# Saguaro-Biosciences/image-processing-suite

Measured on AMD Instinct MI355X. Metric: fields-of-view/sec, 2080x2080x5ch illum+seg+feat pipe, higher is better.
Workload: dtype fp32 planes / fp64 QC+features / fp32 CPnet (split-fp16 MFMA, f16x3); 1 GPU; configs[1]: 384-well plate, 1 FOV/well, 2080x2080x5ch, illum->seg->feat; batch_per_gpu=48, H=2080, W=2080, C=5, cellpose_model=nuclei, cpnet_weights=cpnet_nuclei_synth.pt, tiles_per_fov=9, parallelism=fov-sharded x1, scheduler=static per-rank steps, steps_this_rank=30, batches_in_flight_per_gpu=2

## Files before the change

### image-processing-suite_amd/csrc/capi.hip

```cpp
#include "cpx_internal.h"
#include <stdarg.h>
#include <stdio.h>
#include <new>

static thread_local char g_err[1024] = {0};

void cpx_set_error(const char* fmt, ...) {
  va_list ap;
  va_start(ap, fmt);
  vsnprintf(g_err, sizeof(g_err), fmt, ap);
  va_end(ap);
}

int cpx_hip_fail(hipError_t e, const char* what) {
  cpx_set_error("HIP error %d (%s) in %s", (int)e, hipGetErrorString(e), what);
  (void)hipGetLastError();
  return e == hipErrorOutOfMemory ? CPX_ERR_OOM : CPX_ERR_HIP;
}

void* cpx_ws(cpx_ctx* ctx, int slot, size_t bytes) {
  if (bytes == 0) bytes = 16;
  if (ctx->ws_bytes[slot] >= bytes) return ctx->ws[slot];
  if (ctx->ws[slot]) {
    (void)hipStreamSynchronize(ctx->stream);
    (void)hipFree(ctx->ws[slot]);
    ctx->ws[slot] = nullptr;
    ctx->ws_bytes[slot] = 0;
  }
  size_t want = bytes + bytes / 4;
  void* p = nullptr;
  hipError_t e = hipMalloc(&p, want);
  if (e != hipSuccess) {
    cpx_hip_fail(e, "workspace hipMalloc");
    return nullptr;
  }
  ctx->ws[slot] = p;
  ctx->ws_bytes[slot] = want;
  ++ctx->ws_gen[slot];
  return p;
}

extern "C" {

int cpx_abi_version(void) { return CPX_ABI_VERSION; }

const char* cpx_last_error(void) { return g_err; }

int cpx_init(int device, cpx_ctx** out) {
  CPX_REQUIRE(out != nullptr, CPX_ERR_ARG, "cpx_init: out is NULL");
  g_err[0] = 0;
  int n = 0;
  CPX_CHECK_HIP(hipGetDeviceCount(&n));
  CPX_REQUIRE(device >= 0 && device < n, CPX_ERR_ARG, "cpx_init: device %d of %d", device, n);
  CPX_CHECK_HIP(hipSetDevice(device));
  cpx_ctx* c = new (std::nothrow) cpx_ctx();
  CPX_REQUIRE(c != nullptr, CPX_ERR_OOM, "cpx_init: host allocation failed");
  c->device = device;
  hipError_t e = hipStreamCreateWithFlags(&c->own_stream, hipStreamNonBlocking);
  if (e != hipSuccess) {
    delete c;
    return cpx_hip_fail(e, "hipStreamCreate");
  }
  c->stream = c->own_stream;
  hipDeviceProp_t prop;
  if (hipGetDeviceProperties(&prop, device) == hipSuccess) c->n_cu = prop.multiProcessorCount;
  *out = c;
  return CPX_OK;
}

void cpx_destroy(cpx_ctx* ctx) {
  if (!ctx) return;
  (void)hipSetDevice(ctx->device);
  if (ctx->stream) (void)hipStreamSynchronize(ctx->stream);
  cpx_fov_free(ctx);
  for (int i = 0; i < kWsSlots; ++i)
    if (ctx->ws[i]) (void)hipFree(ctx->ws[i]);
  if (ctx->own_stream) (void)hipStreamDestroy(ctx->own_stream);
  for (int i = 0; i < cpx_ctx::kGlcmEv; ++i)
    for (int k = 0; k < 2; ++k)
      if (ctx->glcm_ev[i][k]) (void)hipEventDestroy(ctx->glcm_ev[i][k]);
  for (int i = 0; i < cpx_ctx::kSegEv; ++i) {
    for (int k = 0; k < 4; ++k)
      if (ctx->seg_ev[i][k]) (void)hipEventDestroy(ctx->seg_ev[i][k]);
    if (ctx->seg_cnt[i]) (void)hipHostFree(ctx->seg_cnt[i]);
  }
  delete ctx;
}

int cpx_debug_glcm_timing(cpx_ctx* ctx, int enable) {
  CPX_REQUIRE(ctx != nullptr, CPX_ERR_ARG, "cpx_debug_glcm_timing: ctx is NULL");
  if (enable && !ctx->glcm_ev[0][0])
    for (int i = 0; i < cpx_ctx::kGlcmEv; ++i)
      for (int k = 0; k < 2; ++k) CPX_CHECK_HIP(hipEventCreate(&ctx->glcm_ev[i][k]));
  ctx->glcm_timing = enable ? 1 : 0;
  ctx->glcm_nev = 0;
  return CPX_OK;
}

int cpx_debug_glcm_ms(cpx_ctx* ctx, double* ms_out, int* launches_out) {
  CPX_REQUIRE(ctx && ms_out, CPX_ERR_ARG, "cpx_debug_glcm_ms: null argument");
  double ms = 0.0;
  for (int i = 0; i < ctx->glcm_nev; ++i) {
    CPX_CHECK_HIP(hipEventSynchronize(ctx->glcm_ev[i][1]));
    float t = 0.0f;
    CPX_CHECK_HIP(hipEventElapsedTime(&t, ctx->glcm_ev[i][0], ctx->glcm_ev[i][1]));
    ms += t;
  }
  *ms_out = ms;
  if (launches_out) *launches_out = ctx->glcm_nev;
  ctx->glcm_nev = 0;
  return CPX_OK;
}

int cpx_debug_seg_timing(cpx_ctx* ctx, int enable) {
  CPX_REQUIRE(ctx != nullptr, CPX_ERR_ARG, "cpx_debug_seg_timing: ctx is NULL");
  if (enable && !ctx->seg_ev[0][0])
    for (int i = 0; i < cpx_ctx::kSegEv; ++i)
      for (int k = 0; k < 4; ++k) CPX_CHECK_HIP(hipEventCreate(&ctx->seg_ev[i][k]));
  ctx->seg_timing = enable ? 1 : 0;
  ctx->seg_nev = 0;
  return CPX_OK;
}

int cpx_debug_seg_stats(cpx_ctx* ctx, double* follow_ms, double* item_steps, double* fe_reg_ms, int* calls) {
  CPX_REQUIRE(ctx && follow_ms && item_steps && fe_reg_ms, CPX_ERR_ARG, "cpx_debug_seg_stats: null argument");
  double fm = 0.0, st = 0.0, fe = 0.0;
  for (int i = 0; i < ctx->seg_nev; ++i) {
    CPX_CHECK_HIP(hipEventSynchronize(ctx->seg_ev[i][3]));
    float t = 0.0f;
    CPX_CHECK_HIP(hipEventElapsedTime(&t, ctx->seg_ev[i][0], ctx->seg_ev[i][1]));
    fm += t;
    CPX_CHECK_HIP(hipEventElapsedTime(&t, ctx->seg_ev[i][2], ctx->seg_ev[i][3]));
    fe += t;
    const int B = ctx->seg_B[i];
    const int* c = ctx->seg_cnt[i];
    for (int r = 0; r < ctx->seg_rounds[i]; ++r)
      for (int b = 0; b < B; ++b) st += (double)c[r * B + b] * ctx->seg_K[i][r];
  }
  *follow_ms = fm;
  *item_steps = st;
  *fe_reg_ms = fe;
  if (calls) *calls = ctx->seg_nev;
  ctx->seg_nev = 0;
  return CPX_OK;
}

int cpx_debug_flow_error_counts(cpx_ctx* ctx, int out[8]) {
  CPX_REQUIRE(ctx && out, CPX_ERR_ARG, "cpx_debug_flow_error_counts: null argument");
  for (int i = 0; i < 8; ++i) out[i] = 0;
  if (ctx->fe_count_off < 0 || !ctx->ws[WS_SEG_OBJ]) return CPX_OK;
  int c[8];
  CPX_CHECK_HIP(hipMemcpyAsync(c, (const unsigned char*)ctx->ws[WS_SEG_OBJ] + ctx->fe_count_off, sizeof(c),
                               hipMemcpyDeviceToHost, ctx->stream));
  CPX_CHECK_HIP(hipStreamSynchronize(ctx->stream));
  for (int i = 0; i < kFeLists; ++i) out[i] = c[i];
  return CPX_OK;
}

int cpx_debug_flow_error_class(int bh, int bw) { return fe_class(bh, bw); }

int cpx_set_stream(cpx_ctx* ctx, void* hip_stream) {
  CPX_REQUIRE(ctx != nullptr, CPX_ERR_ARG, "cpx_set_stream: ctx is NULL");
  ctx->stream = (hipStream_t)hip_stream;
  if (ctx->own_stream && ctx->stream != ctx->own_stream) {
    (void)hipStreamSynchronize(ctx->own_stream);
    (void)hipStreamDestroy(ctx->own_stream);
    ctx->own_stream = nullptr;
  }
  return CPX_OK;
}

int cpx_sync(cpx_ctx* ctx) {
  CPX_REQUIRE(ctx != nullptr, CPX_ERR_ARG, "cpx_sync: ctx is NULL");
  CPX_CHECK_HIP(hipStreamSynchronize(ctx->stream));
  return CPX_OK;
}

int cpx_stream_create_cu_mask(int device, const uint32_t* cu_mask, int n_words, void** out) {
  CPX_REQUIRE(cu_mask && out && n_words > 0, CPX_ERR_ARG, "cpx_stream_create_cu_mask: bad argument");
  int n = 0;
  CPX_CHECK_HIP(hipGetDeviceCount(&n));
  CPX_REQUIRE(device >= 0 && device < n, CPX_ERR_ARG, "cpx_stream_create_cu_mask: device %d of %d", device, n);
  int prev = 0;
  CPX_CHECK_HIP(hipGetDevice(&prev));
  CPX_CHECK_HIP(hipSetDevice(device));
  hipStream_t s = nullptr;
  const hipError_t e = hipExtStreamCreateWithCUMask(&s, (uint32_t)n_words, cu_mask);
  (void)hipSetDevice(prev);
  if (e != hipSuccess) return cpx_hip_fail(e, "hipExtStreamCreateWithCUMask");
  *out = (void*)s;
  return CPX_OK;
}

int cpx_stream_destroy(void* stream) {
  CPX_REQUIRE(stream != nullptr, CPX_ERR_ARG, "cpx_stream_destroy: stream is NULL");
  CPX_CHECK_HIP(hipStreamSynchronize((hipStream_t)stream));
  CPX_CHECK_HIP(hipStreamDestroy((hipStream_t)stream));
  return CPX_OK;
}

}

extern "C" int cpx_reserve(cpx_ctx* ctx, int max_planes, int H, int W, int max_fovs,
                           int max_label) {
  CPX_REQUIRE(ctx != nullptr, CPX_ERR_ARG, "cpx_reserve: ctx is NULL");
  CPX_REQUIRE(max_planes > 0 && H > 0 && W > 0 && max_fovs >= 0 && max_label >= 0, CPX_ERR_ARG,
              "cpx_reserve: bad sizes");
  if (!cpx_ws(ctx, WS_PARTIALS, (size_t)48 * 64 * max_planes)) return CPX_ERR_OOM;
  const int K = std::max(std::min(H, W) / 8, 1);
  const int nr = std::max(K - 2, 1);
  if (!cpx_ws(ctx, WS_QC_ROWS, (size_t)16 * max_planes * H * K)) return CPX_ERR_OOM;
  size_t ring = (size_t)8 * max_planes * K * nr;
  ring = ((ring + 255) / 256) * 256 + (size_t)8 * max_planes + 256;
  if (!cpx_ws(ctx, WS_QC_RINGS, ring)) return CPX_ERR_OOM;
  if (!cpx_ws(ctx, WS_QC_MISC, (size_t)16 * (H + W) + 256)) return CPX_ERR_OOM;
  return CPX_OK;
}
```

### image-processing-suite_amd/csrc/k_seg.hip

```cpp
#include "cpx_internal.h"
#include <stdlib.h>
#include <limits.h>
#include <math.h>
#include <stdio.h>
#include <type_traits>
#include <vector>

#pragma clang fp contract(off)

namespace {

constexpr int kT = 256;
constexpr int kRpad = 20;

__device__ __forceinline__ unsigned int f2key(float f) {
  unsigned int u = __float_as_uint(f);
  return (u & 0x80000000u) ? ~u : (u | 0x80000000u);
}
__device__ __forceinline__ float key2f(unsigned int k) {
  unsigned int u = (k & 0x80000000u) ? (k & 0x7fffffffu) : ~k;
  return __uint_as_float(u);
}
__device__ __forceinline__ unsigned short f2bf16(float f) {
  unsigned int u = __float_as_uint(f);
// ... 198 lines not shown
      static_cast<float*>(tiles)[(ntile * npx + q) * nchan + ch] = out;
    else
      static_cast<unsigned short*>(tiles)[(ntile * npx + q) * nchan + ch] = f2bf16(out);
  }
}

__global__ __launch_bounds__(kT) void k_seg_average(const void* __restrict__ net, int layout, int nout,
                                                    cpx_seg_geom g, const float* __restrict__ taper,
                                                    float* __restrict__ yf) {
  const int fov = blockIdx.y;
  const int q = blockIdx.x * kT + threadIdx.x;
  if (q >= g.Ly * g.Lx) return;
  const int y = q / g.Lx, x = q - y * g.Lx;
  const int py = y + g.py0, px = x + g.px0;
  const int npx = g.by * g.bx;
  float acc[4] = {0.f, 0.f, 0.f, 0.f};
  float nav = 0.0f;
  for (int jy = 0; jy < g.ny; ++jy) {
    const int ty = py - g.ys[jy];
    if (ty < 0 || ty >= g.by) continue;
    for (int jx = 0; jx < g.nx; ++jx) {
      const int tx = px - g.xs[jx];
      if (tx < 0 || tx >= g.bx) continue;
      const long long t = (long long)fov * g.ny * g.nx + jy * g.nx + jx;
      const int o = ty * g.bx + tx;
      const float m = taper[o];
      for (int c = 0; c < nout && c < 4; ++c) {
        float v;
        if (layout == CPX_TILE_F32_NCHW) v = static_cast<const float*>(net)[(t * nout + c) * npx + o];
        else if (layout == CPX_TILE_F32_NHWC) v = static_cast<const float*>(net)[(t * npx + o) * nout + c];
        else v = bf162f(static_cast<const unsigned short*>(net)[(t * npx + o) * nout + c]);
        acc[c] = acc[c] + v * m;
      }
      nav = nav + m;
    }
  }
  for (int c = 0; c < nout && c < 4; ++c)
    yf[(((long long)fov * nout + c) * g.Ly + y) * g.Lx + x] = acc[c] / nav;
}

struct DynBufs {
  float2* dps;
  float2* dpf;
  float2* p;
  unsigned char* mov;
  int* h;
  unsigned int* M;
  unsigned char* sflag;
  int* m0;
  int ms;
  int* seeds;
  int* cnt;
  int* first;
  int* newlab;
  unsigned char* mark;
  int* marklist;
  int* act;
  void* fitems0;
  void* fitems1;
  int* fcnt;
  int* tiles;
  int* totals;
  cpx_seg_stats* st;
};

constexpr int kPrepPer = 8;

template <bool RESAMPLE>
__global__ __launch_bounds__(kT) void k_dyn_prep(const float* __restrict__ yf, int Ly, int Lx,
                                                 int Dy, int Dx, AxisTab uy, AxisTab ux,
                                                 DynBufs d) {
  const int fov = blockIdx.y;
  const long long n = (long long)Dy * Dx;
  const long long nl = (long long)Ly * Lx;
  const long long q0 = (long long)blockIdx.x * kT * kPrepPer;
  const float* f = yf + (long long)fov * 3 * nl;
  unsigned int movbits = 0;
#pragma unroll
  for (int k = 0; k < kPrepPer; ++k) {
    const long long q = q0 + k * kT + threadIdx.x;
    if (q >= n) break;
    float v[3];
    if (RESAMPLE) {
      const int qi = (int)q;
      const int y = qi / Dx, x = qi - y * Dx;
      const int y0 = uy.i0[y], y1 = uy.i1[y], x0 = ux.i0[x], x1 = ux.i1[x];
      const float wy = uy.w[y], wx = ux.w[x];
#pragma unroll
      for (int c = 0; c < 3; ++c) {
        const float* P = f + c * nl;
        const float r0 = P[y0 * Lx + x0] * (1.0f - wx) + P[y0 * Lx + x1] * wx;
        const float r1 = P[y1 * Lx + x0] * (1.0f - wx) + P[y1 * Lx + x1] * wx;
        v[c] = r0 * (1.0f - wy) + r1 * wy;
      }
    } else {
#pragma unroll
      for (int c = 0; c < 3; ++c) v[c] = f[c * nl + q];
    }
    const float cp = v[2] > 0.0f ? 1.0f : 0.0f;
    const float dy = (v[0] * cp) / 5.0f, dx = (v[1] * cp) / 5.0f;
    d.dps[(long long)fov * n + q] = make_float2(dy, dx);
    d.dpf[(long long)fov * n + q] = make_float2(v[0], v[1]);
    const bool moving = fabsf(dy) > 1e-3f;
    d.mov[(long long)fov * n + q] = (unsigned char)moving;
    movbits |= (unsigned int)moving << k;
  }
  __shared__ int wsum[kPrepPer][kT / 64];
  __shared__ int sbase;
  const int lane = threadIdx.x & 63, wid = threadIdx.x >> 6;
  unsigned long long bal[kPrepPer];
#pragma unroll
  for (int k = 0; k < kPrepPer; ++k) {
    bal[k] = __ballot((movbits >> k) & 1u);
    if (lane == 0) wsum[k][wid] = __popcll(bal[k]);
  }
  __syncthreads();
  if (threadIdx.x == 0) {
    int s = 0;
    for (int k = 0; k < kPrepPer; ++k)
      for (int w = 0; w < kT / 64; ++w) {
        const int c = wsum[k][w];
        wsum[k][w] = s;
        s += c;
      }
    sbase = s ? atomicAdd(&d.st[fov].n_moving, s) : 0;
  }
  __syncthreads();
  const unsigned long long lower = (1ull << lane) - 1ull;
#pragma unroll
  for (int k = 0; k < kPrepPer; ++k)
    if ((movbits >> k) & 1u)
      d.act[(long long)fov * n + sbase + wsum[k][wid] + __popcll(bal[k] & lower)] =
          (int)(q0 + k * kT + threadIdx.x);
}

__device__ __forceinline__ void agg_add(int* base, int key, bool valid) {
  const int lane = threadIdx.x & 63;
  unsigned long long pend = __ballot(valid);
  while (pend) {
    const int leader = __ffsll((long long)pend) - 1;
    const int k0 = __shfl(key, leader);
    const unsigned long long m = __ballot(valid && key == k0);
    if (lane == leader) atomicAdd(&base[k0], __popcll(m));
    pend &= ~m;
  }
}

struct FollowItem {
  int q;
  float py, px;
  int pad;
};

template <int NI, bool V4>
__global__ __launch_bounds__(kT) void k_dyn_follow(int Dy, int Dx, int niter, int step0, int K,
                                                   int from_act, const FollowItem* __restrict__ in,
                                                   const int* __restrict__ in_cnt,
                                                   FollowItem* __restrict__ out,
                                                   int* __restrict__ out_cnt, DynBufs d) {
  const int fov = blockIdx.y;
  const long long n = (long long)Dy * Dx;
  const int n_moving = d.st[fov].n_moving;
  if (n_moving < 5) return;
  const int n_in = from_act ? n_moving : in_cnt[fov];
  const int steps = min(K, niter - step0);
  const float2* __restrict__ I = d.dps + (long long)fov * n;
  float2* __restrict__ P = d.p + (long long)fov * n;
  const FollowItem* src = in + (long long)fov * n;
  FollowItem* dst = out + (long long)fov * n;
  const float fLy = (float)(Dy - 1), fLx = (float)(Dx - 1);
  const int lane = threadIdx.x & 63, wid = threadIdx.x >> 6;
  const int Dxh = Dx + 2 * kRpad;
  int* Hh = d.h + (long long)fov * (Dy + 2 * kRpad) * Dxh;
  const unsigned char* Ib = reinterpret_cast<const unsigned char*>(I);
  const __amdgpu_buffer_rsrc_t rsI =
      __builtin_amdgcn_make_buffer_rsrc(const_cast<float2*>(I), (short)0, (int)(8 * n), 0x00020000);
  (void)rsI;
  __shared__ int wsum[NI][kT / 64];
  __shared__ int sbase;
  for (int i0 = blockIdx.x * kT * NI; i0 < n_in; i0 += gridDim.x * kT * NI) {
    bool active[NI], done[NI];
    int q[NI];
    float py[NI], px[NI];
#pragma unroll
    for (int j = 0; j < NI; ++j) {
      const int i = i0 + j * kT + threadIdx.x;
      active[j] = i < n_in;
      q[j] = 0;
      py[j] = 0.0f;
      px[j] = 0.0f;
      if (active[j]) {
        if (from_act) {
          q[j] = d.act[(long long)fov * n + i];
          py[j] = (float)(q[j] / Dx);
          px[j] = (float)(q[j] % Dx);
        } else {
          const FollowItem it = src[i];
          q[j] = it.q;
          py[j] = it.py;
          px[j] = it.px;
        }
      }
      done[j] = !active[j];
    }
    float2 af[NI], bf[NI], cf[NI], ef[NI];
    int cy[NI], cx[NI];
#pragma unroll
    for (int j = 0; j < NI; ++j) {
      cy[j] = -1;
      cx[j] = -1;
      af[j] = bf[j] = cf[j] = ef[j] = make_float2(0.0f, 0.0f);
    }
    for (int s = 0; s < steps; ++s) {
      bool all = true;
#pragma unroll
      for (int j = 0; j < NI; ++j) all = all && done[j];
      if (all) break;
      int yi[NI], xi[NI];
#pragma unroll
      for (int j = 0; j < NI; ++j) {
        yi[j] = (int)py[j];
        xi[j] = (int)px[j];
        if (yi[j] == cy[j] && xi[j] == cx[j]) continue;
        cy[j] = yi[j];
        cx[j] = xi[j];
        const int y0 = min(Dy - 1, max(0, yi[j])), x0 = min(Dx - 1, max(0, xi[j]));
        const unsigned int b00 = 8u * (unsigned int)(y0 * Dx + x0);
        const unsigned int bdx = x0 + 1 < Dx ? 8u : 0u, bdy = y0 + 1 < Dy ? 8u * (unsigned int)Dx : 0u;
        if constexpr (V4) {
          const unsigned int o = bdx ? b00 : b00 - 8u;
          const float4 r0 = __builtin_bit_cast(float4, __builtin_amdgcn_raw_buffer_load_b128(rsI, o, 0, 0));
          const float4 r1 = __builtin_bit_cast(float4, __builtin_amdgcn_raw_buffer_load_b128(rsI, o + bdy, 0, 0));
          af[j] = bdx ? make_float2(r0.x, r0.y) : make_float2(r0.z, r0.w);
          bf[j] = make_float2(r0.z, r0.w);
          cf[j] = bdx ? make_float2(r1.x, r1.y) : make_float2(r1.z, r1.w);
          ef[j] = make_float2(r1.z, r1.w);
        } else {
          af[j] = *reinterpret_cast<const float2*>(Ib + b00);
          bf[j] = *reinterpret_cast<const float2*>(Ib + (b00 + bdx));
          cf[j] = *reinterpret_cast<const float2*>(Ib + (b00 + bdy));
          ef[j] = *reinterpret_cast<const float2*>(Ib + (b00 + bdy + bdx));
        }
      }
#pragma unroll
      for (int j = 0; j < NI; ++j) {
        const double2 a = {(double)af[j].x, (double)af[j].y}, b = {(double)bf[j].x, (double)bf[j].y},
                      c = {(double)cf[j].x, (double)cf[j].y}, e = {(double)ef[j].x, (double)ef[j].y};
        double vy, vx;
        if (py[j] >= 1.0f && px[j] >= 1.0f) {
          const float yf = py[j] - (float)yi[j], xf = px[j] - (float)xi[j];
          const double y1 = (double)yf, x1 = (double)xf, y0d = (double)(1.0f - yf), x0d = (double)(1.0f - xf);
          const double w00 = y0d * x0d, w01 = y0d * x1, w10 = y1 * x0d, w11 = y1 * x1;
          vy = a.x * w00 + b.x * w01 + c.x * w10 + e.x * w11;
          vx = a.y * w00 + b.y * w01 + c.y * w10 + e.y * w11;
        } else {
          const double yy = (double)py[j] - (double)yi[j], xx = (double)px[j] - (double)xi[j];
          vy = a.x * (1.0 - yy) * (1.0 - xx) + b.x * (1.0 - yy) * xx + c.x * yy * (1.0 - xx) + e.x * yy * xx;
          vx = a.y * (1.0 - yy) * (1.0 - xx) + b.y * (1.0 - yy) * xx + c.y * yy * (1.0 - xx) + e.y * yy * xx;
        }
        const float ny = __builtin_amdgcn_fmed3f(py[j] + (float)vy, 0.0f, fLy);
        const float nx = __builtin_amdgcn_fmed3f(px[j] + (float)vx, 0.0f, fLx);
        if (!done[j]) {
          if (ny == py[j] && nx == px[j]) done[j] = true;
          py[j] = ny;
          px[j] = nx;
        }
      }
    }
    const bool last = step0 + steps >= niter;
    bool carry[NI];
    unsigned long long bal[NI];
#pragma unroll
    for (int j = 0; j < NI; ++j) {
      const bool fin = active[j] && (done[j] || last);
      agg_add(Hh, ((int)py[j] + kRpad) * Dxh + (int)px[j] + kRpad, fin);
    }
#pragma unroll
    for (int j = 0; j < NI; ++j) {
      if (active[j] && (done[j] || last)) P[q[j]] = make_float2(py[j], px[j]);
      carry[j] = active[j] && !done[j] && !last;
      bal[j] = __ballot(carry[j]);
      if (lane == 0) wsum[j][wid] = __popcll(bal[j]);
    }
    __syncthreads();
    if (threadIdx.x == 0) {
      int t = 0;
      for (int j = 0; j < NI; ++j)
        for (int w = 0; w < kT / 64; ++w) {
          const int c = wsum[j][w];
          wsum[j][w] = t;
          t += c;
        }
      sbase = t ? atomicAdd(&out_cnt[fov], t) : 0;
    }
    __syncthreads();
#pragma unroll
    for (int j = 0; j < NI; ++j)
      if (carry[j]) {
        FollowItem it;
        it.q = q[j];
        it.py = py[j];
        it.px = px[j];
        it.pad = 0;
        dst[sbase + wsum[j][wid] + __popcll(bal[j] & ((1ull << lane) - 1ull))] = it;
      }
    __syncthreads();
  }
}

constexpr int kPx4 = 4;

__global__ __launch_bounds__(kT) void k_hist_init(int Dy, int Dx, DynBufs d) {
  const int fov = blockIdx.y;
  const int Dxh = Dx + 2 * kRpad, Dyh = Dy + 2 * kRpad;
  const long long nh = (long long)Dyh * Dxh;
  const long long b0 = ((long long)blockIdx.x * kT + threadIdx.x) * kPx4;
  if (b0 >= nh) return;
  const unsigned char* mov = d.mov + (long long)fov * Dy * Dx;
  int v[kPx4];
#pragma unroll
  for (int u = 0; u < kPx4; ++u) {
    const long long b = b0 + u;
    v[u] = 0;
    if (b < nh) {
      const int bi = (int)b;
      const int y = bi / Dxh - kRpad, x = bi - (bi / Dxh) * Dxh - kRpad;
      if (y >= 0 && y < Dy && x >= 0 && x < Dx) v[u] = mov[(long long)y * Dx + x] ? 0 : 1;
    }
  }
  int* h = d.h + (long long)fov * nh;
  if ((nh & 3) == 0) {
    *reinterpret_cast<int4*>(h + b0) = make_int4(v[0], v[1], v[2], v[3]);
  } else {
#pragma unroll
    for (int u = 0; u < kPx4; ++u)
      if (b0 + u < nh) h[b0 + u] = v[u];
  }
}

__global__ __launch_bounds__(kT) void k_hist_moving(int Dy, int Dx, DynBufs d) {
  const int fov = blockIdx.y;
  const long long n = (long long)Dy * Dx;
  const int i = blockIdx.x * kT + threadIdx.x;
  const int n_moving = d.st[fov].n_moving;
  if (n_moving >= 5 || (long long)blockIdx.x * kT >= n_moving) return;
  const int Dxh = Dx + 2 * kRpad;
  const bool valid = i < n_moving;
  int key = 0;
  if (valid) {
    const int q = d.act[(long long)fov * n + i];
    float2 pp = n_moving >= 5 ? d.p[(long long)fov * n + q] : make_float2((float)(q / Dx), (float)(q % Dx));
    key = ((int)pp.x + kRpad) * Dxh + (int)pp.y + kRpad;
  }
  agg_add(d.h + (long long)fov * (Dy + 2 * kRpad) * Dxh, key, valid);
}

__global__ __launch_bounds__(kT) void k_seed_flags(int Dyh, int Dxh, DynBufs d) {
  const int fov = blockIdx.y;
  const long long nh = (long long)Dyh * Dxh;
  const long long q0 = ((long long)blockIdx.x * kT + threadIdx.x) * kPx4;
  if (q0 >= nh) return;
  const int* h = d.h + (long long)fov * nh;
  const bool vec = (nh & 3) == 0;
  int v[kPx4];
  if (vec) {
    const int4 t = *reinterpret_cast<const int4*>(h + q0);
    v[0] = t.x;
    v[1] = t.y;
    v[2] = t.z;
    v[3] = t.w;
  } else {
#pragma unroll
    for (int u = 0; u < kPx4; ++u) v[u] = q0 + u < nh ? h[q0 + u] : 0;
  }
  unsigned int fw = 0;
#pragma unroll
  for (int u = 0; u < kPx4; ++u) {
    if (v[u] <= 10) continue;
    const long long q = q0 + u;
    const int y = (int)(q / Dxh), x = (int)(q % Dxh);
    int mx = v[u];
    for (int dy = -2; dy <= 2; ++dy)
      for (int dx = -2; dx <= 2; ++dx) {
        int yy = y + dy, xx = x + dx;
        yy = yy < 0 ? -yy - 1 : (yy >= Dyh ? 2 * Dyh - yy - 1 : yy);
        xx = xx < 0 ? -xx - 1 : (xx >= Dxh ? 2 * Dxh - xx - 1 : xx);
        mx = max(mx, h[(long long)yy * Dxh + xx]);
      }
    fw |= (unsigned int)(v[u] >= mx) << (8 * u);
  }
  unsigned char* f = d.sflag + (long long)fov * nh;
  if (vec && ((((uintptr_t)(f + q0)) & 3u) == 0)) {
    *reinterpret_cast<unsigned int*>(f + q0) = fw;
  } else {
#pragma unroll
    for (int u = 0; u < kPx4; ++u)
      if (q0 + u < nh) f[q0 + u] = (unsigned char)((fw >> (8 * u)) & 1u);
  }
}

constexpr int kOcThreads = 256;
constexpr int kOcPer = 32;
constexpr int kOcTile = kOcThreads * kOcPer;

__device__ __forceinline__ int oc_load(const unsigned char* f, long long n, long long i0,
                                       unsigned int* bits) {
  unsigned int b = 0;
  if (i0 + kOcPer <= n && (((uintptr_t)(f + i0)) & 15u) == 0) {
    const uint4* v = reinterpret_cast<const uint4*>(f + i0);
#pragma unroll
    for (int h = 0; h < 2; ++h) {
      const uint4 t = v[h];
      const unsigned int w[4] = {t.x, t.y, t.z, t.w};
#pragma unroll
      for (int k = 0; k < 4; ++k)
#pragma unroll
        for (int by = 0; by < 4; ++by)
          b |= (((w[k] >> (8 * by)) & 0xffu) ? 1u : 0u) << (h * 16 + k * 4 + by);
    }
  } else {
    for (int j = 0; j < kOcPer; ++j)
      if (i0 + j < n && f[i0 + j]) b |= 1u << j;
  }
  *bits = b;
  return __popc(b);
}

__global__ __launch_bounds__(kOcThreads) void k_oc_count(const unsigned char* __restrict__ flags,
                                                         long long n, int ntile, int* __restrict__ tiles) {
  const int fov = blockIdx.y, t = blockIdx.x;
  const unsigned char* f = flags + (long long)fov * n;
  unsigned int bits;
  int c = oc_load(f, n, (long long)t * kOcTile + (long long)threadIdx.x * kOcPer, &bits);
  c = wave_sum(c);
  __shared__ int ws[kOcThreads / 64];
  if ((threadIdx.x & 63) == 0) ws[threadIdx.x >> 6] = c;
  __syncthreads();
  if (threadIdx.x == 0) {
    int s = 0;
    for (int w = 0; w < kOcThreads / 64; ++w) s += ws[w];
    tiles[(long long)fov * ntile + t] = s;
  }
}

__global__ __launch_bounds__(1024) void k_oc_scan(int ntile, int* __restrict__ tiles,
                                                  int* __restrict__ totals) {
  const int fov = blockIdx.x;
  int* t = tiles + (long long)fov * ntile;
  __shared__ int wsum[16];
  __shared__ int base;
  if (threadIdx.x == 0) base = 0;
  __syncthreads();
  const int lane = threadIdx.x & 63, wid = threadIdx.x >> 6;
  for (int i0 = 0; i0 < ntile; i0 += 1024) {
    const int i = i0 + threadIdx.x;
    const int v = i < ntile ? t[i] : 0;
    int inc = v;
// ... 1453 lines not shown
  if (!buf) return CPX_ERR_OOM;
  int* base = (int*)buf;
  t.ty.i0 = base;
  t.ty.i1 = base + Ly;
  t.ty.w = (const float*)(base + 2 * Ly);
  t.tx.i0 = base + 3 * Ly;
  t.tx.i1 = base + 3 * Ly + Lx;
  t.tx.w = (const float*)(base + 3 * Ly + 2 * Lx);
  t.ynear = base + 3 * Ly + 3 * Lx;
  t.xnear = base + 3 * Ly + 3 * Lx + H;
  int* up = base + 3 * Ly + 3 * Lx + H + W;
  t.uy.i0 = up;
  t.uy.i1 = up + H;
  t.uy.w = (const float*)(up + 2 * H);
  t.ux.i0 = up + 3 * H;
  t.ux.i1 = up + 3 * H + W;
  t.ux.w = (const float*)(up + 3 * H + 2 * W);
  const int key[6] = {H, W, Ly, Lx, 2, 0};
  bool same = ctx->seg_gen == ctx->ws_gen[WS_SEG_TAB];
  for (int i = 0; i < 6; ++i) same = same && ctx->seg_key[i] == key[i];
  if (same) return CPX_OK;
  std::vector<int> h(words);
  axis_coeffs(H, Ly, &h[0], &h[Ly], (float*)&h[2 * Ly]);
  axis_coeffs(W, Lx, &h[3 * Ly], &h[3 * Ly + Lx], (float*)&h[3 * Ly + 2 * Lx]);
  const double ify = 1.0 / ((double)H / (double)Ly), ifx = 1.0 / ((double)W / (double)Lx);
  for (int y = 0; y < H; ++y) h[3 * Ly + 3 * Lx + y] = std::min((int)floor(y * ify), Ly - 1);
  for (int x = 0; x < W; ++x) h[3 * Ly + 3 * Lx + H + x] = std::min((int)floor(x * ifx), Lx - 1);
  const size_t u = (size_t)3 * Ly + 3 * Lx + H + W;
  axis_coeffs(Ly, H, &h[u], &h[u + H], (float*)&h[u + 2 * H]);
  axis_coeffs(Lx, W, &h[u + 3 * H], &h[u + 3 * H + W], (float*)&h[u + 3 * H + 2 * W]);
  CPX_CHECK_HIP(hipMemcpyAsync(buf, h.data(), words * 4, hipMemcpyHostToDevice, ctx->stream));
  CPX_CHECK_HIP(hipStreamSynchronize(ctx->stream));
  for (int i = 0; i < 6; ++i) ctx->seg_key[i] = key[i];
  ctx->seg_gen = ctx->ws_gen[WS_SEG_TAB];
  return CPX_OK;
}

bool geom_ok(const cpx_seg_geom* g) {
  if (!g || g->Ly <= 0 || g->Lx <= 0 || g->by <= 0 || g->bx <= 0) return false;
  if (g->ny < 1 || g->nx < 1 || g->ny > CPX_SEG_MAX_TILES_AXIS || g->nx > CPX_SEG_MAX_TILES_AXIS) return false;
  for (int i = 0; i < g->ny; ++i)
    if (g->ys[i] < 0 || g->ys[i] + g->by > g->Lyp) return false;
  for (int i = 0; i < g->nx; ++i)
    if (g->xs[i] < 0 || g->xs[i] + g->bx > g->Lxp) return false;
  return g->py0 >= 0 && g->px0 >= 0 && g->py0 + g->Ly <= g->Lyp && g->px0 + g->Lx <= g->Lxp;
}

}

extern "C" int cpx_seg_percentiles(cpx_ctx* ctx, const float* corr_dev, int B, int C, int H, int W,
                                   int nchan, double* pct_dev) {
  CPX_REQUIRE(ctx && corr_dev && pct_dev, CPX_ERR_ARG, "cpx_seg_percentiles: null argument");
  CPX_REQUIRE(B > 0 && C > 0 && nchan > 0 && nchan <= C && H > 0 && W > 0 && B * nchan <= 65535,
              CPX_ERR_ARG, "cpx_seg_percentiles: bad sizes");
  const int P = B * nchan;
  const size_t hist_bytes = (size_t)P * 4 * 2048 * 4;
  unsigned char* ws = (unsigned char*)cpx_ws(ctx, WS_SEG_PCT, hist_bytes + sizeof(PctState) * P + 256);
  if (!ws) return CPX_ERR_OOM;
  unsigned int* hist = (unsigned int*)ws;
  PctState* st = (PctState*)(ws + hist_bytes);
  const long long N = (long long)H * W;
  for (int pass = 0; pass < 3; ++pass) {
    CPX_CHECK_HIP(hipMemsetAsync(hist, 0, hist_bytes, ctx->stream));
    hipLaunchKernelGGL(k_pct_hist, dim3(48, P), dim3(kT), 0, ctx->stream, corr_dev, C, N, nchan,
                       pass, (const PctState*)st, hist);
    CPX_CHECK_LAUNCH("k_pct_hist");
    hipLaunchKernelGGL(k_pct_find, dim3(P), dim3(256), 0, ctx->stream, N, pass, st,
                       (const unsigned int*)hist, pct_dev);
    CPX_CHECK_LAUNCH("k_pct_find");
  }
  return CPX_OK;
}

extern "C" int cpx_seg_tiles(cpx_ctx* ctx, const float* corr_dev, int B, int C, int H, int W,
                             int nchan, const double* pct_dev, const cpx_seg_geom* geom, int layout,
                             void* tiles_dev) {
  CPX_REQUIRE(ctx && corr_dev && pct_dev && tiles_dev, CPX_ERR_ARG, "cpx_seg_tiles: null argument");
  CPX_REQUIRE(geom_ok(geom), CPX_ERR_ARG, "cpx_seg_tiles: bad geometry");
  CPX_REQUIRE(B > 0 && B <= 65535 && nchan > 0 && nchan <= C && H > 0 && W > 0, CPX_ERR_ARG,
              "cpx_seg_tiles: bad sizes");
  CPX_REQUIRE(layout == CPX_TILE_F32_NCHW || layout == CPX_TILE_BF16_NHWC || layout == CPX_TILE_F32_NHWC,
              CPX_ERR_ARG, "cpx_seg_tiles: bad layout %d", layout);
  SegTabs t;
  int rc = seg_tables(ctx, H, W, geom->Ly, geom->Lx, t);
  if (rc) return rc;
  const int npx = geom->by * geom->bx;
  hipLaunchKernelGGL(k_seg_tiles, dim3(cpx_div_up(npx, kT), geom->ny * geom->nx, B), dim3(kT), 0,
                     ctx->stream, corr_dev, C, H, W, nchan, pct_dev, *geom, t.ty, t.tx, layout,
                     tiles_dev);
  CPX_CHECK_LAUNCH("k_seg_tiles");
  return CPX_OK;
}

extern "C" int cpx_seg_average(cpx_ctx* ctx, const void* net_dev, int layout, int B, int nout,
                               const cpx_seg_geom* geom, const float* taper_dev, float* yf_dev) {
  CPX_REQUIRE(ctx && net_dev && taper_dev && yf_dev, CPX_ERR_ARG, "cpx_seg_average: null argument");
  CPX_REQUIRE(geom_ok(geom), CPX_ERR_ARG, "cpx_seg_average: bad geometry");
  CPX_REQUIRE(B > 0 && B <= 65535 && nout > 0 && nout <= 4, CPX_ERR_ARG, "cpx_seg_average: bad sizes");
  hipLaunchKernelGGL(k_seg_average, dim3(cpx_div_up(geom->Ly * geom->Lx, kT), B), dim3(kT), 0,
                     ctx->stream, net_dev, layout, nout, *geom, taper_dev, yf_dev);
  CPX_CHECK_LAUNCH("k_seg_average");
  return CPX_OK;
}

static int ordered_compact(cpx_ctx* ctx, const unsigned char* flags, long long n, int B, int* tiles,
                           int* totals, int cap, int* out, long long out_stride) {
  const int ntile = cpx_div_up(n, kOcTile);
  hipLaunchKernelGGL(k_oc_count, dim3(ntile, B), dim3(kOcThreads), 0, ctx->stream, flags, n, ntile, tiles);
  hipLaunchKernelGGL(k_oc_scan, dim3(B), dim3(1024), 0, ctx->stream, ntile, tiles, totals);
  hipLaunchKernelGGL(k_oc_emit, dim3(ntile, B), dim3(kOcThreads), 0, ctx->stream, flags, n, ntile,
                     (const int*)tiles, cap, out, out_stride);
  CPX_CHECK_LAUNCH("ordered_compact");
  return CPX_OK;
}

__global__ void k_seed_count(int B, int ms, const int* __restrict__ totals, cpx_seg_stats* __restrict__ st) {
  const int fov = blockIdx.x * blockDim.x + threadIdx.x;
  if (fov >= B) return;
  const int t = totals[fov];
  st[fov].n_seeds = min(t, ms);
  st[fov].n_seeds_found = t;
  if (t > ms) atomicOr(&st[fov].overflow, CPX_SEG_OVF_SEEDS);
}

extern "C" int cpx_seg_masks(cpx_ctx* ctx, const float* yf_dev, int B, const cpx_seg_geom* geom,
                             int H, int W, int niter, double flow_threshold, int min_size,
                             int max_objects, int resample, int32_t* labels_dev,
                             cpx_seg_stats* stats_dev) {
  CPX_REQUIRE(ctx && yf_dev && labels_dev && stats_dev, CPX_ERR_ARG, "cpx_seg_masks: null argument");
  CPX_REQUIRE(geom_ok(geom), CPX_ERR_ARG, "cpx_seg_masks: bad geometry");
  CPX_REQUIRE(B > 0 && B <= 65535 && H > 0 && W > 0 && niter >= 0 && max_objects > 0 &&
                  (long long)(H + 2 * kRpad) * (W + 2 * kRpad) < (1LL << 31) &&
                  (long long)H * W * (long long)sizeof(float2) < (1LL << 32),
              CPX_ERR_ARG, "cpx_seg_masks: bad sizes");
  const int Ly = geom->Ly, Lx = geom->Lx;
  const int Dy = resample ? H : Ly, Dx = resample ? W : Lx;
  const int Dyh = Dy + 2 * kRpad, Dxh = Dx + 2 * kRpad;
  const long long n = (long long)Dy * Dx, nh = (long long)Dyh * Dxh;
  SegTabs tabs;
  int rc = seg_tables(ctx, H, W, Ly, Lx, tabs);
  if (rc) return rc;
  auto al = [](size_t b) { return (b + 255) / 256 * 256; };
  const int ntile = cpx_div_up(std::max(n, nh), kOcTile);
  const size_t sz_f2 = al(sizeof(float2) * B * n);
  const size_t sz_d2 = al(sizeof(float2) * B * n);
  const size_t sz_b = al((size_t)B * n);
  const size_t sz_h = al(sizeof(int) * B * nh), sz_hb = al((size_t)B * nh);
  const size_t sz_m0 = resample ? 0 : al(sizeof(int) * B * n);
  const int ms = max_objects;
  const size_t sz_seeds = al(sizeof(int) * (size_t)B * ms);
  const size_t sz_cnt = al(sizeof(int) * (size_t)B * (ms + 1));
  const size_t sz_act = al(sizeof(int) * B * n);
  const size_t sz_small = al(sizeof(int) * (size_t)B);
  constexpr int k0 = 16, sw = 384, k1 = 128;
  const int rounds = cpx_div_up(sw, k0) + cpx_div_up(std::max(0, niter - sw), k1) + 2;
  const size_t sz_fcnt = al(sizeof(int) * (size_t)B * (rounds + 1));
  const size_t sz_items = al((size_t)16 * B * n);
  const size_t sz_tiles = al(sizeof(int) * (size_t)B * ntile);
  const size_t total = sz_d2 + 2 * sz_f2 + 2 * sz_b + 2 * sz_h + sz_hb + sz_m0 + 2 * sz_seeds + 3 * sz_cnt +
                       sz_act + sz_small + sz_tiles + sz_fcnt + 2 * sz_items;
  unsigned char* w = (unsigned char*)cpx_ws(ctx, WS_SEG_DYN, total);
  if (!w) return CPX_ERR_OOM;
  DynBufs d;
  d.dps = (float2*)w; w += sz_d2;
  d.dpf = (float2*)w; w += sz_f2;
  d.p = (float2*)w; w += sz_f2;
  d.mov = w; w += sz_b;
  d.mark = w; w += sz_b;
  d.h = (int*)w; w += sz_h;
  d.M = (unsigned int*)w; w += sz_h;
  d.sflag = w; w += sz_hb;
  d.m0 = resample ? labels_dev : (int*)w; w += sz_m0;
  d.seeds = (int*)w; w += sz_seeds;
  d.marklist = (int*)w; w += sz_seeds;
  d.cnt = (int*)w; w += sz_cnt;
  d.first = (int*)w; w += sz_cnt;
  d.newlab = (int*)w; w += sz_cnt;
  d.act = (int*)w; w += sz_act;
  d.fcnt = (int*)w; w += sz_fcnt;
  d.fitems0 = w; w += sz_items;
  d.fitems1 = w; w += sz_items;
  d.totals = (int*)w; w += sz_small;
  d.tiles = (int*)w; w += sz_tiles;
  d.st = stats_dev;
  d.ms = ms;
  CPX_CHECK_HIP(hipMemsetAsync(stats_dev, 0, sizeof(cpx_seg_stats) * B, ctx->stream));
  CPX_CHECK_HIP(hipMemsetAsync(d.M, 0, sz_h, ctx->stream));
  CPX_CHECK_HIP(hipMemsetAsync(d.mark, 0, sz_b, ctx->stream));
  CPX_CHECK_HIP(hipMemsetAsync(d.cnt, 0, sz_cnt, ctx->stream));
  CPX_CHECK_HIP(hipMemsetAsync(d.first, 0x7f, sz_cnt, ctx->stream));
  CPX_CHECK_HIP(hipMemsetAsync(d.newlab, 0, sz_cnt, ctx->stream));
  CPX_CHECK_HIP(hipMemsetAsync(d.fcnt, 0, sz_fcnt, ctx->stream));
  const dim3 gp(cpx_div_up(n, kT), B), gh(cpx_div_up(nh, kT), B);
  const dim3 gprep(cpx_div_up(n, (long long)kT * kPrepPer), B);
  if (resample)
    hipLaunchKernelGGL(k_dyn_prep<true>, gprep, dim3(kT), 0, ctx->stream, yf_dev, Ly, Lx, Dy, Dx,
                       tabs.uy, tabs.ux, d);
  else
    hipLaunchKernelGGL(k_dyn_prep<false>, gprep, dim3(kT), 0, ctx->stream, yf_dev, Ly, Lx, Dy, Dx,
                       tabs.uy, tabs.ux, d);
  const dim3 gh4(cpx_div_up(nh, (long long)kT * kPx4), B), gp4(cpx_div_up(n, (long long)kT * kPx4), B);
  hipLaunchKernelGGL(k_hist_init, gh4, dim3(kT), 0, ctx->stream, Dy, Dx, d);
  const int sev = ctx->seg_timing && ctx->seg_nev < cpx_ctx::kSegEv ? ctx->seg_nev++ : -1;
  bool fe_timed = false;
  if (sev >= 0) CPX_CHECK_HIP(hipEventRecord(ctx->seg_ev[sev][0], ctx->stream));
  {
    const int fblk = std::max(1, std::min(cpx_div_up(n, kT), (16 * ctx->n_cu + B - 1) / B));
    int step = 0, r = 0;
    do {
      const int K = step < sw ? k0 : k1;
      const FollowItem* in = (const FollowItem*)(r & 1 ? d.fitems1 : d.fitems0);
      FollowItem* out = (FollowItem*)(r & 1 ? d.fitems0 : d.fitems1);
      const bool v4 = Dx >= 2 && 8LL * n < (1LL << 31);
      auto kern = v4 ? k_dyn_follow<2, true> : k_dyn_follow<2, false>;
      hipLaunchKernelGGL(kern, dim3(fblk, B), dim3(kT), 0, ctx->stream, Dy, Dx, niter, step, K,
                         r == 0 ? 1 : 0, in, (const int*)(d.fcnt + (size_t)B * r), out,
                         d.fcnt + (size_t)B * (r + 1), d);
      if (sev >= 0 && r < 64) ctx->seg_K[sev][r] = std::min(K, std::max(niter - step, 0));
      step += K;
      ++r;
    } while (step < niter);
    if (sev >= 0) {
      CPX_CHECK_HIP(hipEventRecord(ctx->seg_ev[sev][1], ctx->stream));
      const int rr = std::min(r, 64);
      const int need = B * rr;
      if (ctx->seg_cnt_cap[sev] < need) {
        if (ctx->seg_cnt[sev]) CPX_CHECK_HIP(hipHostFree(ctx->seg_cnt[sev]));
        CPX_CHECK_HIP(hipHostMalloc((void**)&ctx->seg_cnt[sev], sizeof(int) * need));
        ctx->seg_cnt_cap[sev] = need;
      }
      CPX_CHECK_HIP(hipMemcpy2DAsync(ctx->seg_cnt[sev], sizeof(int), stats_dev, sizeof(cpx_seg_stats),
                                     sizeof(int), B, hipMemcpyDeviceToHost, ctx->stream));
      if (rr > 1)
        CPX_CHECK_HIP(hipMemcpyAsync(ctx->seg_cnt[sev] + B, d.fcnt + B, sizeof(int) * B * (rr - 1),
                                     hipMemcpyDeviceToHost, ctx->stream));
      ctx->seg_B[sev] = B;
      ctx->seg_rounds[sev] = rr;
    }
  }
  hipLaunchKernelGGL(k_hist_moving, dim3(1, B), dim3(kT), 0, ctx->stream, Dy, Dx, d);
  hipLaunchKernelGGL(k_seed_flags, gh4, dim3(kT), 0, ctx->stream, Dyh, Dxh, d);
  CPX_CHECK_LAUNCH("cpx_seg_masks follow");
  rc = ordered_compact(ctx, d.sflag, nh, B, d.tiles, d.totals, ms, d.seeds, ms);
  if (rc) return rc;
  hipLaunchKernelGGL(k_seed_count, dim3(cpx_div_up(B, 256)), dim3(256), 0, ctx->stream, B, ms,
                     (const int*)d.totals, stats_dev);
  hipLaunchKernelGGL(k_seed_expand, dim3(std::max(1, (4 * ctx->n_cu + B - 1) / B), B), dim3(kT), 0,
                     ctx->stream, Dyh, Dxh, d);
  hipLaunchKernelGGL(k_assign, dim3(cpx_div_up(n, (long long)kT * kAsg), B), dim3(kT), 0, ctx->stream, Dy, Dx, d);
  hipLaunchKernelGGL(k_relabel_mark, dim3(cpx_div_up(ms, kT), B), dim3(kT), 0, ctx->stream, Dy, Dx, d);
  CPX_CHECK_LAUNCH("cpx_seg_masks seeds");
  rc = ordered_compact(ctx, d.mark, n, B, d.tiles, d.totals, ms, d.marklist, ms);
  if (rc) return rc;
  hipLaunchKernelGGL(k_relabel_apply, dim3(4, B), dim3(kT), 0, ctx->stream, Dy, Dx, d);
  hipLaunchKernelGGL(k_apply_newlab, gp4, dim3(kT), 0, ctx->stream, Dy, Dx, d);
  CPX_CHECK_LAUNCH("cpx_seg_masks relabel");
  const int ML = max_objects;
  const size_t sz_lst = al(sizeof(cpx_label_stats) * (size_t)B * (ML + 1));
  const size_t sz_obj = al(sizeof(cpx_object) * (size_t)B * ML);
  const size_t sz_hdr = al(sizeof(cpx_fov_objects) * (size_t)B);
  const size_t sz_bad = al((size_t)B * (ML + 1));
  const size_t sz_l2i = al(sizeof(int) * (size_t)B * (ML + 1));
  const size_t sz_abs = al(sizeof(int) * (size_t)B * ML);
  const size_t sz_nl = sz_abs;
  constexpr int kFeQueues = 6;
  const size_t sz_fec = al(sizeof(int) * (8 + kFeQueues));
  const size_t sz_fel = al(sizeof(int2) * (size_t)kFeLists * B * ML);
  const size_t gscr_per = (size_t)2 * (Dy + 2) * (Dx + 2);
  const size_t sz_gscr = al(sizeof(double) * B * gscr_per);
  unsigned char* o = (unsigned char*)cpx_ws(ctx, WS_SEG_OBJ,
      sz_lst + sz_obj + sz_hdr + sz_bad + sz_l2i + sz_abs + sz_nl + sz_fec + sz_fel + sz_gscr);
  if (!o) return CPX_ERR_OOM;
  cpx_label_stats* lst = (cpx_label_stats*)o; o += sz_lst;
  cpx_object* obj = (cpx_object*)o; o += sz_obj;
  cpx_fov_objects* hdr = (cpx_fov_objects*)o; o += sz_hdr;
  unsigned char* bad = o; o += sz_bad;
  int* l2i = (int*)o; o += sz_l2i;
  int* absorber = (int*)o; o += sz_abs;
  int* newlab = (int*)o; o += sz_nl;
  int* fec = (int*)o; o += sz_fec;
  int2* fel = (int2*)o; o += sz_fel;
  double* gscr = (double*)o;
  ctx->fe_count_off = -1;
  if (flow_threshold > 0.0) {
    rc = cpx_objects(ctx, d.m0, B, Dy, Dx, ML, 0, lst, obj, hdr);
    if (rc) return rc;
    CPX_CHECK_HIP(hipMemsetAsync(bad, 0, sz_bad, ctx->stream));
    CPX_CHECK_HIP(hipMemsetAsync(fec, 0, sizeof(int) * (8 + kFeQueues), ctx->stream));
    const cpx_fe_lists lists = {fec, fel, (long long)B * ML};
    int* const fq = fec + 8;
    ctx->fe_count_off = (unsigned char*)fec - (unsigned char*)ctx->ws[WS_SEG_OBJ];
    hipLaunchKernelGGL(k_fe_classify, dim3(cpx_div_up(ML, 256), B), dim3(256), 0, ctx->stream, ML,
                       (const cpx_object*)obj, (const cpx_fov_objects*)hdr, lists);
    if (sev >= 0) CPX_CHECK_HIP(hipEventRecord(ctx->seg_ev[sev][2], ctx->stream));
    rc = cpx_flow_error_reg_launch(ctx->n_cu, ctx->stream, d.m0, (const float2*)d.dpf, Dy, Dx, ML, obj, lists,
                                   fq, flow_threshold, bad);
    if (rc) return rc;
    if (sev >= 0) {
      CPX_CHECK_HIP(hipEventRecord(ctx->seg_ev[sev][3], ctx->stream));
      fe_timed = true;
    }
    hipLaunchKernelGGL((k_flow_error_lds<kFeLargeThreads / 2, kFeLargeCells, 2 * kFeU, float, 4>),
                       dim3(2 * ctx->n_cu), dim3(kFeLargeThreads / 2), 0, ctx->stream, (const int*)d.m0,
                       (const float2*)d.dpf, Dy, Dx, ML, (const cpx_object*)obj, lists, fq + 3, flow_threshold,
                       bad);
    hipLaunchKernelGGL(k_flow_error_tail, dim3(ctx->n_cu), dim3(kFeLargeThreads), 0, ctx->stream,
                       (const int*)d.m0, (const float2*)d.dpf, Dy, Dx, ML, (const cpx_object*)obj, lists,
                       fq + 4, flow_threshold, bad);
    {
      const int nbig = std::max(1, std::min(ctx->n_cu, 4 * B));
      const long long slice = (long long)(B * gscr_per / nbig) & ~1LL;
      hipLaunchKernelGGL(k_flow_error_big, dim3(nbig), dim3(kBigThreads), 0, ctx->stream,
                         (const int*)d.m0, (const float2*)d.dpf, Dy, Dx, ML, (const cpx_object*)obj, lists,
                         fq + 5, flow_threshold, gscr, slice, bad);
    }
    hipLaunchKernelGGL(k_flow_error_fov, dim3(B), dim3(kFlowThreads), 0, ctx->stream,
                       (const int*)d.m0, (const float2*)d.dpf, Dy, Dx, ML, (const cpx_object*)obj, lists,
                       flow_threshold, gscr, (long long)gscr_per, bad);
    hipLaunchKernelGGL(k_apply_bad, gp4, dim3(kT), 0, ctx->stream, n, ML,
                       (const unsigned char*)bad, d.m0);
    hipLaunchKernelGGL(k_count_bad, dim3(B), dim3(256), 0, ctx->stream, ML,
                       (const unsigned char*)bad, (const int*)fq, kFeQueues, stats_dev);
    CPX_CHECK_LAUNCH("cpx_seg_masks flow error");
  }
  if (!resample) {
    hipLaunchKernelGGL(k_upsample, dim3(cpx_div_up(W, kT), cpx_div_up(H, kUpRows), B), dim3(kT), 0,
                       ctx->stream, (const int*)d.m0, Ly, Lx, H, W, tabs.ynear, tabs.xnear, labels_dev);
    CPX_CHECK_LAUNCH("k_upsample");
  }
  rc = cpx_objects(ctx, labels_dev, B, H, W, ML, 0, lst, obj, hdr);
  if (rc) return rc;
  const long long N = (long long)H * W;
  const size_t sz_fill = al(sizeof(int) * (size_t)B * N);
  const size_t sz_fscr = al(sizeof(unsigned int) * 2 * (size_t)B * ((W + 31) / 32) * H);
  unsigned char* fw = (unsigned char*)cpx_ws(ctx, WS_SEG_FILL, sz_fill + sz_fscr);
  if (!fw) return CPX_ERR_OOM;
  int* fillidx = (int*)fw;
  unsigned int* fscr = (unsigned int*)(fw + sz_fill);
  CPX_CHECK_HIP(hipMemsetAsync(fillidx, 0, sizeof(int) * (size_t)B * N, ctx->stream));
  CPX_CHECK_HIP(hipMemsetAsync(absorber, 0x7f, sz_abs, ctx->stream));
  CPX_CHECK_HIP(hipMemsetAsync(l2i, 0, sz_l2i, ctx->stream));
  hipLaunchKernelGGL(k_lab2idx, dim3(cpx_div_up(ML, kT), B), dim3(kT), 0, ctx->stream, ML,
                     (const cpx_object*)obj, (const cpx_fov_objects*)hdr, l2i);
  static bool fattr = false;
  const size_t flds = sizeof(unsigned int) * 2 * kFillMaxWords;
  if (!fattr) {
    CPX_CHECK_HIP(hipFuncSetAttribute((const void*)k_fill_holes,
                                      hipFuncAttributeMaxDynamicSharedMemorySize, (int)flds));
    CPX_CHECK_HIP(hipFuncSetAttribute((const void*)k_fill_seq,
                                      hipFuncAttributeMaxDynamicSharedMemorySize, (int)flds));
    fattr = true;
  }
  hipLaunchKernelGGL(k_fill_holes, dim3(std::max(1, std::min(ML, (2 * ctx->n_cu + B - 1) / B)), B),
                     dim3(kFillThreads), flds, ctx->stream,
                     (const int*)labels_dev, H, W, ML, min_size, (const cpx_object*)obj,
                     (const cpx_fov_objects*)hdr, (const int*)l2i, fillidx, absorber);
  hipLaunchKernelGGL(k_fill_holes_big, dim3(B), dim3(1024), 0, ctx->stream,
                     (const int*)labels_dev, H, W, ML, min_size, (const cpx_object*)obj,
                     (const cpx_fov_objects*)hdr, (const int*)l2i, fillidx, absorber, fscr);
  if (sev >= 0 && !fe_timed) {
    CPX_CHECK_HIP(hipEventRecord(ctx->seg_ev[sev][2], ctx->stream));
    CPX_CHECK_HIP(hipEventRecord(ctx->seg_ev[sev][3], ctx->stream));
  }
  hipLaunchKernelGGL(k_fill_final, dim3(B), dim3(1024), 0, ctx->stream, ML, min_size,
                     (const cpx_object*)obj, (const cpx_fov_objects*)hdr, (const int*)absorber,
                     (const int*)labels_dev, (const int*)fillidx, W, N, newlab, stats_dev);
  hipLaunchKernelGGL(k_fill_apply, dim3(std::max(1, std::min(cpx_div_up(N, kT), 8 * ctx->n_cu / B + 1)), B),
// ... 9 lines not shown
```

Baseline: 501.6 FOV/s.

## Restructure Cellpose flow-follow loop with wave ballots, packed loads and occupancy bound

Reworks the per-step flow-following kernel. Per-thread done flags become wave-level ballot masks so the loop exits once no lane in the wave is moving. Bilinear samples are kept in two float4 registers and reloaded only when the cell index changes, with the V4 path dropping clamping in favour of __umul24 address math and a wave-uniform right-edge fixup. The kernel gets a launch-bounds minimum-waves hint and uses mbcnt for compaction offsets. This aims to cut VALU work, redundant loads and register pressure in the hot iteration, but relies on positions staying in range, since the clamp is removed, and the occupancy hint may cause spills.

```diff
diff --git a/image-processing-suite_amd/csrc/capi.hip b/image-processing-suite_amd/csrc/capi.hip
--- a/image-processing-suite_amd/csrc/capi.hip
+++ b/image-processing-suite_amd/csrc/capi.hip
@@ -117,6 +117,7 @@
   if (enable && !ctx->seg_ev[0][0])
     for (int i = 0; i < cpx_ctx::kSegEv; ++i)
       for (int k = 0; k < 4; ++k) CPX_CHECK_HIP(hipEventCreate(&ctx->seg_ev[i][k]));
+  for (int i = 0; i < ctx->seg_nev; ++i) CPX_CHECK_HIP(hipEventSynchronize(ctx->seg_ev[i][3]));
   ctx->seg_timing = enable ? 1 : 0;
   ctx->seg_nev = 0;
   return CPX_OK;
diff --git a/image-processing-suite_amd/csrc/k_seg.hip b/image-processing-suite_amd/csrc/k_seg.hip
--- a/image-processing-suite_amd/csrc/k_seg.hip
+++ b/image-processing-suite_amd/csrc/k_seg.hip
@@ -374,13 +374,24 @@
   int pad;
 };
 
+typedef float FollowQuad __attribute__((ext_vector_type(4)));
+
+#ifndef CPX_FOLLOW_NI
+#define CPX_FOLLOW_NI 2
+#endif
+#ifndef CPX_FOLLOW_K0
+#define CPX_FOLLOW_K0 16
+#endif
+#ifndef CPX_FOLLOW_WAVES
+#define CPX_FOLLOW_WAVES 8
+#endif
+
 template <int NI, bool V4>
-__global__ __launch_bounds__(kT) void k_dyn_follow(int Dy, int Dx, int niter, int step0, int K,
-                                                   int from_act, const FollowItem* __restrict__ in,
-                                                   const int* __restrict__ in_cnt,
-                                                   FollowItem* __restrict__ out,
-                                                   int* __restrict__ out_cnt, DynBufs d) {
+__global__ __launch_bounds__(kT, V4 ? CPX_FOLLOW_WAVES : 1) void k_dyn_follow(
+    int Dy, int Dx, int niter, int step0, int K, int from_act, const FollowItem* __restrict__ in,
+    const int* __restrict__ in_cnt, FollowItem* __restrict__ out, int* __restrict__ out_cnt, DynBufs d) {
   const int fov = blockIdx.y;
+  const int bx = blockIdx.x, nbx = gridDim.x;
   const long long n = (long long)Dy * Dx;
   const int n_moving = d.st[fov].n_moving;
   if (n_moving < 5) return;
@@ -391,6 +402,8 @@
   const FollowItem* src = in + (long long)fov * n;
   FollowItem* dst = out + (long long)fov * n;
   const float fLy = (float)(Dy - 1), fLx = (float)(Dx - 1);
+  const int Dym1 = Dy - 1, Dxm1 = Dx - 1;
+  const unsigned int Dx8 = 8u * (unsigned int)Dx;
   const int lane = threadIdx.x & 63, wid = threadIdx.x >> 6;
   const int Dxh = Dx + 2 * kRpad;
   int* Hh = d.h + (long long)fov * (Dy + 2 * kRpad) * Dxh;
@@ -400,10 +413,11 @@
   (void)rsI;
   __shared__ int wsum[NI][kT / 64];
   __shared__ int sbase;
-  for (int i0 = blockIdx.x * kT * NI; i0 < n_in; i0 += gridDim.x * kT * NI) {
-    bool active[NI], done[NI];
+  for (int i0 = bx * kT * NI; i0 < n_in; i0 += nbx * kT * NI) {
+    bool active[NI];
     int q[NI];
     float py[NI], px[NI];
+    unsigned long long moving[NI], act[NI];
 #pragma unroll
     for (int j = 0; j < NI; ++j) {
       const int i = i0 + j * kT + threadIdx.x;
@@ -423,54 +437,78 @@
           px[j] = it.px;
         }
       }
-      done[j] = !active[j];
-    }
-    float2 af[NI], bf[NI], cf[NI], ef[NI];
-    int cy[NI], cx[NI];
+      act[j] = moving[j] = __ballot(active[j]);
+    }
+    FollowQuad r0[NI], r1[NI];
+    unsigned int cb[NI];
 #pragma unroll
     for (int j = 0; j < NI; ++j) {
-      cy[j] = -1;
-      cx[j] = -1;
-      af[j] = bf[j] = cf[j] = ef[j] = make_float2(0.0f, 0.0f);
+      cb[j] = 0xffffffffu;
+      r0[j] = r1[j] = FollowQuad{0.0f, 0.0f, 0.0f, 0.0f};
     }
     for (int s = 0; s < steps; ++s) {
-      bool all = true;
-#pragma unroll
-      for (int j = 0; j < NI; ++j) all = all && done[j];
-      if (all) break;
+      unsigned long long any = 0;
+#pragma unroll
+      for (int j = 0; j < NI; ++j) any |= moving[j];
+      if (any == 0) break;
       int yi[NI], xi[NI];
+      unsigned int o0[NI], o1[NI];
+      bool changed[NI], redge[NI];
 #pragma unroll
       for (int j = 0; j < NI; ++j) {
         yi[j] = (int)py[j];
         xi[j] = (int)px[j];
-        if (yi[j] == cy[j] && xi[j] == cx[j]) continue;
-        cy[j] = yi[j];
-        cx[j] = xi[j];
-        const int y0 = min(Dy - 1, max(0, yi[j])), x0 = min(Dx - 1, max(0, xi[j]));
-        const unsigned int b00 = 8u * (unsigned int)(y0 * Dx + x0);
-        const unsigned int bdx = x0 + 1 < Dx ? 8u : 0u, bdy = y0 + 1 < Dy ? 8u * (unsigned int)Dx : 0u;
+        unsigned int b00;
+        int y0 = yi[j], x0 = xi[j];
         if constexpr (V4) {
-          const unsigned int o = bdx ? b00 : b00 - 8u;
-          const float4 r0 = __builtin_bit_cast(float4, __builtin_amdgcn_raw_buffer_load_b128(rsI, o, 0, 0));
-          const float4 r1 = __builtin_bit_cast(float4, __builtin_amdgcn_raw_buffer_load_b128(rsI, o + bdy, 0, 0));
-          af[j] = bdx ? make_float2(r0.x, r0.y) : make_float2(r0.z, r0.w);
-          bf[j] = make_float2(r0.z, r0.w);
-          cf[j] = bdx ? make_float2(r1.x, r1.y) : make_float2(r1.z, r1.w);
-          ef[j] = make_float2(r1.z, r1.w);
+          b00 = 8u * (__umul24((unsigned int)y0, (unsigned int)Dx) + (unsigned int)x0);
         } else {
-          af[j] = *reinterpret_cast<const float2*>(Ib + b00);
-          bf[j] = *reinterpret_cast<const float2*>(Ib + (b00 + bdx));
-          cf[j] = *reinterpret_cast<const float2*>(Ib + (b00 + bdy));
-          ef[j] = *reinterpret_cast<const float2*>(Ib + (b00 + bdy + bdx));
+          y0 = min(Dy - 1, max(0, y0));
+          x0 = min(Dx - 1, max(0, x0));
+          b00 = 8u * (unsigned int)(y0 * Dx + x0);
         }
+        changed[j] = b00 != cb[j];
+        cb[j] = b00;
+        redge[j] = x0 >= Dxm1;
+        o0[j] = (V4 && redge[j]) ? b00 - 8u : b00;
+        o1[j] = y0 < Dym1 ? o0[j] + Dx8 : o0[j];
       }
 #pragma unroll
       for (int j = 0; j < NI; ++j) {
-        const double2 a = {(double)af[j].x, (double)af[j].y}, b = {(double)bf[j].x, (double)bf[j].y},
-                      c = {(double)cf[j].x, (double)cf[j].y}, e = {(double)ef[j].x, (double)ef[j].y};
+        if (!changed[j]) continue;
+        if constexpr (V4) {
+          r0[j] = __builtin_bit_cast(FollowQuad, __builtin_amdgcn_raw_buffer_load_b128(rsI, o0[j], 0, 0));
+          r1[j] = __builtin_bit_cast(FollowQuad, __builtin_amdgcn_raw_buffer_load_b128(rsI, o1[j], 0, 0));
+        } else {
+          const unsigned int bdx = redge[j] ? 0u : 8u;
+          const float2 a = *reinterpret_cast<const float2*>(Ib + o0[j]);
+          const float2 b = *reinterpret_cast<const float2*>(Ib + (o0[j] + bdx));
+          const float2 c = *reinterpret_cast<const float2*>(Ib + o1[j]);
+          const float2 e = *reinterpret_cast<const float2*>(Ib + (o1[j] + bdx));
+          r0[j] = FollowQuad{a.x, a.y, b.x, b.y};
+          r1[j] = FollowQuad{c.x, c.y, e.x, e.y};
+        }
+      }
+#pragma unroll
+      for (int j = 0; j < NI; ++j) asm volatile("" : "+v"(r0[j]), "+v"(r1[j]));
+#pragma unroll
+      for (int j = 0; j < NI; ++j) {
+        if constexpr (V4) {
+          if (__builtin_amdgcn_ballot_w64(px[j] >= fLx) != 0) {
+            asm volatile("" : "+v"(r0[j]), "+v"(r1[j]));
+            if (px[j] >= fLx) {
+              r0[j].x = r0[j].z;
+              r0[j].y = r0[j].w;
+              r1[j].x = r1[j].z;
+              r1[j].y = r1[j].w;
+            }
+          }
+        }
+        const double2 a = {(double)r0[j].x, (double)r0[j].y}, b = {(double)r0[j].z, (double)r0[j].w},
+                      c = {(double)r1[j].x, (double)r1[j].y}, e = {(double)r1[j].z, (double)r1[j].w};
         double vy, vx;
         if (py[j] >= 1.0f && px[j] >= 1.0f) {
-          const float yf = py[j] - (float)yi[j], xf = px[j] - (float)xi[j];
+          const float yf = __builtin_amdgcn_fractf(py[j]), xf = __builtin_amdgcn_fractf(px[j]);
           const double y1 = (double)yf, x1 = (double)xf, y0d = (double)(1.0f - yf), x0d = (double)(1.0f - xf);
           const double w00 = y0d * x0d, w01 = y0d * x1, w10 = y1 * x0d, w11 = y1 * x1;
           vy = a.x * w00 + b.x * w01 + c.x * w10 + e.x * w11;
@@ -482,13 +520,15 @@
         }
         const float ny = __builtin_amdgcn_fmed3f(py[j] + (float)vy, 0.0f, fLy);
         const float nx = __builtin_amdgcn_fmed3f(px[j] + (float)vx, 0.0f, fLx);
-        if (!done[j]) {
-          if (ny == py[j] && nx == px[j]) done[j] = true;
-          py[j] = ny;
-          px[j] = nx;
-        }
-      }
-    }
+        moving[j] = (__builtin_amdgcn_ballot_w64(ny != py[j]) | __builtin_amdgcn_ballot_w64(nx != px[j])) &
+                    act[j];
+        py[j] = ny;
+        px[j] = nx;
+      }
+    }
+    bool done[NI];
+#pragma unroll
+    for (int j = 0; j < NI; ++j) done[j] = !((moving[j] >> lane) & 1ull);
     const bool last = step0 + steps >= niter;
     bool carry[NI];
     unsigned long long bal[NI];
@@ -524,7 +564,9 @@
         it.py = py[j];
         it.px = px[j];
         it.pad = 0;
-        dst[sbase + wsum[j][wid] + __popcll(bal[j] & ((1ull << lane) - 1ull))] = it;
+        const int below = (int)__builtin_amdgcn_mbcnt_hi((unsigned int)(bal[j] >> 32),
+                                                         __builtin_amdgcn_mbcnt_lo((unsigned int)bal[j], 0u));
+        dst[sbase + wsum[j][wid] + below] = it;
       }
     __syncthreads();
   }
@@ -2284,7 +2326,7 @@
   const size_t sz_cnt = al(sizeof(int) * (size_t)B * (ms + 1));
   const size_t sz_act = al(sizeof(int) * B * n);
   const size_t sz_small = al(sizeof(int) * (size_t)B);
-  constexpr int k0 = 16, sw = 384, k1 = 128;
+  constexpr int k0 = CPX_FOLLOW_K0, sw = 384, k1 = 128;
   const int rounds = cpx_div_up(sw, k0) + cpx_div_up(std::max(0, niter - sw), k1) + 2;
   const size_t sz_fcnt = al(sizeof(int) * (size_t)B * (rounds + 1));
   const size_t sz_items = al((size_t)16 * B * n);
@@ -2343,8 +2385,8 @@
       const int K = step < sw ? k0 : k1;
       const FollowItem* in = (const FollowItem*)(r & 1 ? d.fitems1 : d.fitems0);
       FollowItem* out = (FollowItem*)(r & 1 ? d.fitems0 : d.fitems1);
-      const bool v4 = Dx >= 2 && 8LL * n < (1LL << 31);
-      auto kern = v4 ? k_dyn_follow<2, true> : k_dyn_follow<2, false>;
+      const bool v4 = Dx >= 2 && 8LL * n < (1LL << 31) && Dy <= (1 << 24) && Dx <= (1 << 24);
+      auto kern = v4 ? k_dyn_follow<CPX_FOLLOW_NI, true> : k_dyn_follow<2, false>;
       hipLaunchKernelGGL(kern, dim3(fblk, B), dim3(kT), 0, ctx->stream, Dy, Dx, niter, step, K,
                          r == 0 ? 1 : 0, in, (const int*)(d.fcnt + (size_t)B * r), out,
                          d.fcnt + (size_t)B * (r + 1), d);
```

Measured after the change: 510.2 FOV/s (median of 6 runs). 1.02x the previous value.
